# timmeinhardt/trackformer

Measured on AMD Instinct MI355X. Metric: frames/sec, TrackFormer-Deformable inference (ResNet-50, 1333x800, 300 object + 100 track queries, bs 1 per GPU); roofline = ms_deform_attn HBM GB/s, higher is better.
Workload: dtype f32 (dense layers as the fp16 split product on MFMA: two fp16 pieces per activation, three per weight scaled per output channel -- 22 + 1 significand bits per operand, the one dropped product < 2^-22 --, three terms, f32 accumulate)

## Files before the change

include/tf_fused.h:

```cpp
#ifndef TF_FUSED_H_
#define TF_FUSED_H_

#include <stdint.h>

#ifdef __cplusplus
extern "C" {
#endif

int tf_bias_act_f32(float *x, const float *bias, const float *residual, int64_t n, int C, int relu,
                    void *stream);

int tf_add_layernorm_f32(const float *x, const float *res, const float *gamma, const float *beta,
                         float *out, int64_t rows, int C, float eps, void *stream);

int tf_box_refine_f32(const float *delta, const float *ref, float *out, int64_t rows, int ref_dim, float eps, void *stream);

int tf_postprocess_pack_f32(const float *logits, const float *boxes, float *out, int64_t Q, int C, float img_h, float img_w,
                            int clip, void *stream);

int tf_groupnorm_nhwc_f32(const float *x, const float *gamma, const float *beta, float *out, double *workspace, int N,
                          int HW, int C, int G, float eps, int64_t x_image_stride, int64_t out_image_stride, void *stream);
int tf_groupnorm_stats_nhwc_f32(const float *x, double *workspace, int N, int HW, int C, int G, int64_t x_image_stride, void *stream);
int tf_groupnorm_relu_nhwc_f32(const float *x, const float *gamma, const float *beta, float *out, double *workspace, int N,
                               int HW, int C, int G, float eps, int64_t x_image_stride, int64_t out_image_stride, void *stream);

int tf_upsample_add_nhwc_f32(const float *low, const float *fpn, float *out, int N, int q_per_image, int h, int w, int H, int W, int C,
                             void *stream);

int tf_conv3x3_merge_packed_f32(const float *low, const float *fpn, const double *gn_workspace, const float *gamma, const float *beta,
                                int groups, float eps, const void *w_packed, const float *bias, float *y, int nimg, int q_per_image, int lh,
                                int lw, int H, int W, int cin, int cout, int relu, int terms, void *stream);

int tf_groupnorm_relu_conv3x3_c1_nhwc_f32(const float *x, const float *gamma, const float *beta, const float *weight, float bias,
                                          float *out, double *workspace, int N, int H, int W, int C, int G, float eps, void *stream);

int tf_mask_label_map_f32(const float *logits, const int *order, int16_t *label, int n_tracks, int h, int w, int pad_h, int pad_w, int img_h,
                          int img_w, int out_h, int out_w, float threshold, void *stream);


// ... 87 lines not shown
```

include/tf_msda.h:

```cpp
#ifndef TF_MSDA_H_
#define TF_MSDA_H_

#include <stdint.h>

#ifdef __cplusplus
extern "C" {
#endif

#define TF_MSDA_ABI_VERSION 8
#define TF_MSDA_MAX_LEVELS 16

typedef enum tf_msda_status {
    TF_MSDA_OK = 0,
    TF_MSDA_ERR_NULL_POINTER = -1,
    TF_MSDA_ERR_BAD_DIMS = -2,
    TF_MSDA_ERR_SHAPE_SUM = -3,
    TF_MSDA_ERR_LAUNCH = -4,
    TF_MSDA_ERR_NO_DEVICE = -5,
    TF_MSDA_ERR_WORKSPACE = -6
} tf_msda_status;

int tf_msda_abi_version(void);

const char *tf_msda_strerror(int status);
// ... 87 lines not shown
```

trackformer_amd/_cabi.py:

```python
import ctypes
import os

_PKG_DIR = os.path.dirname(os.path.abspath(__file__))
LIB_PATH = os.environ.get("TF_MSDA_LIB") or os.path.join(_PKG_DIR, "lib", "libtf_msda.so")

EXPORTED_SYMBOLS = (
    "tf_msda_abi_version",
    "tf_msda_strerror",
    "tf_msda_last_hip_error",
    "tf_msda_last_kernel",
    "tf_msda_set_tiled",
    "tf_msda_set_option",
    "tf_msda_debug_trace_buffer",
    "tf_msda_forward_fused_f32",
    "tf_msda_forward_f32",
    "tf_msda_forward_f64",
    "tf_msda_forward_f32_dshapes",
    "tf_msda_forward_f64_dshapes",
    "tf_msda_backward_f32",
    "tf_msda_backward_f64",
    "tf_msda_backward_f32_dshapes",
    "tf_msda_backward_f64_dshapes",
    "tf_msda_backward_det_workspace_bytes",
    "tf_msda_backward_det_f32",
    "tf_msda_backward_det_f64",
    "tf_msda_backward_det_f32_dshapes",
    "tf_msda_backward_det_f64_dshapes",
    "tf_msda_fused_prologue_f32",
    "tf_msda_fused_backward_epilogue_f32",
    "tf_msda_forward_host_f32",
    "tf_msda_forward_host_f64",
    "tf_msda_backward_host_f32",
    "tf_msda_backward_host_f64",
    "tf_bias_act_f32",
    "tf_add_layernorm_f32",
    "tf_groupnorm_nhwc_f32",
    "tf_groupnorm_relu_nhwc_f32",
    "tf_box_refine_f32",
    "tf_postprocess_pack_f32",
    "tf_upsample_add_nhwc_f32",
    "tf_mask_label_map_f32",
    "tf_conv3x3_merge_packed_f32",
    "tf_groupnorm_stats_nhwc_f32",
    "tf_groupnorm_relu_conv3x3_c1_nhwc_f32",
    "tf_bias_relu_maxpool_f32",
    "tf_stem_conv7x7_f32",
    "tf_linear_split_f32",
    "tf_linear_split_res_f32",
    "tf_conv3x3_split_f32",
    "tf_conv3x3_splitk_f32",
    "tf_conv1x1_strided_split_f32",
    "tf_conv1x1_splitk_f32",
# ... 8 lines not shown
    "tf_add_layernorm_train_f32",
    "tf_add_layernorm_bwd_workspace_bytes",
    "tf_add_layernorm_bwd_f32",
    "tf_set_criterion_fwd_f32",
    "tf_set_criterion_bwd_f32",
    "tf_match_cost_f32",
    "tf_linear_split_add_f32",
    "tf_ffn_fused_f32",
    "tf_linear_res_ln_f32",
    "tf_linear_groups_f32",
    "tf_conv_packed_f32",
    "tf_mha_core_f32",
    "tf_nms_host_f32",
)

ABI_VERSION = 8

_lib = None


class ProjGroup(ctypes.Structure):
    _fields_ = [("w_packed", ctypes.c_void_p), ("bias", ctypes.c_void_p), ("y", ctypes.c_void_p), ("N", ctypes.c_int),
                ("add_x2", ctypes.c_int)]


class MSDAError(RuntimeError):
    """Raised when libtf_msda.so reports a non-zero status."""


def lib():
    global _lib
# ... 61 lines not shown
    L.tf_postprocess_pack_f32.restype = ci
    L.tf_postprocess_pack_f32.argtypes = [vp, vp, vp, ctypes.c_int64, ci, ctypes.c_float, ctypes.c_float, ci, vp]
    L.tf_groupnorm_stats_nhwc_f32.restype = ci
    L.tf_groupnorm_stats_nhwc_f32.argtypes = [vp, vp, ci, ci, ci, ci, ctypes.c_int64, vp]
    L.tf_conv3x3_merge_packed_f32.restype = ci
    L.tf_conv3x3_merge_packed_f32.argtypes = [vp, vp, vp, vp, vp, ci, ctypes.c_float, vp, vp, vp, ci, ci, ci, ci, ci, ci, ci, ci, ci, ci, vp]
    L.tf_mask_label_map_f32.restype = ci
    L.tf_mask_label_map_f32.argtypes = [vp, vp, vp, ci, ci, ci, ci, ci, ci, ci, ci, ci, ctypes.c_float, vp]
    L.tf_upsample_add_nhwc_f32.restype = ci
    L.tf_upsample_add_nhwc_f32.argtypes = [vp, vp, vp, ci, ci, ci, ci, ci, ci, ci, vp]
    L.tf_groupnorm_relu_conv3x3_c1_nhwc_f32.restype = ci
    L.tf_groupnorm_relu_conv3x3_c1_nhwc_f32.argtypes = [vp, vp, vp, vp, ctypes.c_float, vp, vp, ci, ci, ci, ci, ci, ctypes.c_float, vp]
    for fn in (L.tf_groupnorm_nhwc_f32, L.tf_groupnorm_relu_nhwc_f32):
        fn.restype = ci
        fn.argtypes = [vp, vp, vp, vp, vp, ci, ci, ci, ci, ctypes.c_float, ctypes.c_int64, ctypes.c_int64, vp]
    L.tf_linear_split_f32.restype = ci
    L.tf_linear_split_f32.argtypes = [vp, vp, vp, vp, vp, vp, vp, ctypes.c_int64, ci, ci, ci, vp]
    L.tf_linear_split_res_f32.restype = ci
    L.tf_linear_split_res_f32.argtypes = [vp, vp, vp, vp, vp, vp, vp, vp, ctypes.c_int64, ci, ci, ci, vp]
    L.tf_conv3x3_splitk_f32.restype = ci
    L.tf_conv3x3_splitk_f32.argtypes = [vp, vp, vp, vp, vp, vp, vp, vp, ci, ci, ci, ci, ci, ci, ci, ci, vp]
    L.tf_conv3x3_split_f32.restype = ci
    L.tf_conv3x3_split_f32.argtypes = [vp, vp, vp, vp, vp, vp, vp] + [ci] * 7 + [vp]
    L.tf_conv1x1_splitk_f32.restype = ci
    L.tf_conv1x1_splitk_f32.argtypes = [vp, vp, vp, vp, vp, vp, vp, vp, ci, ci, ci, ci, ci, ci, ci, ci, vp]
    L.tf_conv1x1_strided_split_f32.restype = ci
    L.tf_conv1x1_strided_split_f32.argtypes = [vp, vp, vp, vp, vp, vp, vp] + [ci] * 7 + [vp]
    L.tf_linear_packed_bytes.restype = ctypes.c_int64
    L.tf_linear_packed_bytes.argtypes = [ci, ci, ci]
    L.tf_linear_pack_weight_f32.restype = ci
# ... 53 lines not shown
```

trackformer_amd/backbone.py:

```python
from collections import OrderedDict
from typing import Dict, List

import torch
import torch.nn.functional as F
from torch import nn

from . import fused
from .nested import NestedTensor, all_valid_mask, is_all_valid
from .position_encoding import build_position_encoding


import os as _os

CHANNELS_LAST = _os.environ.get("TF_BACKBONE_NCHW", "0") != "1"


_conv1x1_split = _os.environ.get("TF_CONV1X1_SPLIT", "1") != "0"


_conv3x3_split = _os.environ.get("TF_CONV3X3_SPLIT", "1") != "0"


def _parse_skip(text):
    out = set()
# ... 240 lines not shown
                return y
            y = y + b.reshape(1, -1, 1, 1)
        else:
            y = F.conv2d(x, cache.weight, b, conv.stride, conv.padding, conv.dilation, conv.groups)
        if residual is not None:
            y = y.add_(residual)
        return F.relu_(y) if relu else y
    if fold == 2 and not x.is_cuda:
        fold = 0
    x = bn(conv(x))
    if residual is not None:
        x = x + residual
    return F.relu(x) if relu else x


def _stem_pooled(x, conv1, bn1, maxpool, cache: _FoldCache):
    if not ((fused.stem_pool_fused_enabled() or fused.stem_conv_split_enabled()) and x.is_cuda and CHANNELS_LAST
            and isinstance(bn1, FrozenBatchNorm2d)
            and isinstance(maxpool, nn.MaxPool2d) and maxpool.kernel_size == 3 and maxpool.stride == 2
            and maxpool.padding == 1 and maxpool.dilation == 1 and not maxpool.ceil_mode):
        return None
    b = cache.get(conv1, bn1)
    w = cache.weight
    y = None
    if (conv1.kernel_size == (7, 7) and conv1.stride == (2, 2) and conv1.padding == (3, 3) and conv1.dilation == (1, 1)
            and conv1.groups == 1):
        fuse_pool = fused.stem_pool_fused_enabled()
        y = fused.stem_conv(x, w, None if fuse_pool else b, relu=not fuse_pool)
        if y is not None and not fuse_pool:
            return maxpool(y)
    if y is None:
        if not fused.stem_pool_fused_enabled():
            return None
        y = F.conv2d(x, w, None, conv1.stride, conv1.padding, conv1.dilation, conv1.groups)
    pooled = fused.bias_relu_maxpool(y, b)
    if pooled is None:
        if fused.bias_act_(y, b, None, True) is None:
            y = F.relu_(y + b.reshape(1, -1, 1, 1))
        pooled = maxpool(y)
    return pooled


class Bottleneck(nn.Module):
    expansion = 4

    def __init__(self, inplanes, planes, stride=1, downsample=None, dilation=1,
                 norm_layer=FrozenBatchNorm2d):
        super().__init__()
# ... 96 lines not shown

    def __init__(self, model: nn.Module, return_layers: Dict[str, str]):
        if not set(return_layers).issubset(name for name, _ in model.named_children()):
            raise ValueError("return_layers are not present in model")
        remaining = dict(return_layers)
        kept = OrderedDict()
        for name, module in model.named_children():
            kept[name] = module
            remaining.pop(name, None)
            if not remaining:
                break
        super().__init__(kept)
        self.return_layers = dict(return_layers)
        self._fold = _FoldCache()

    def forward(self, x):
        out = OrderedDict()
        fold = _fold_mode(self["conv1"], x) if (self.training and "conv1" in self) else int(_inference_mode(self))
        fused_stem = fold == 1 and all(k in self for k in ("conv1", "bn1", "relu"))
        pooled_stem = (fused_stem and "maxpool" in self
                       and not any(k in self.return_layers for k in ("conv1", "bn1", "relu", "maxpool")))
        skip = ()
        for name, module in self.items():
            if name in skip or (fused_stem and name in ("bn1", "relu")):
                continue
            if fused_stem and name == "conv1":
                pooled = _stem_pooled(x, self["conv1"], self["bn1"], self["maxpool"], self._fold) if pooled_stem else None
                if pooled is not None:
                    x, skip = pooled, ("maxpool",)
                    continue
                x = _conv_bn(x, self["conv1"], self["bn1"], self._fold, True, 1)
            else:
                x = module(x)
            if name in self.return_layers:
                out[self.return_layers[name]] = x
        return out


class BackboneBase(nn.Module):
    def __init__(self, backbone: nn.Module, train_backbone: bool, return_interm_layers: bool):
        super().__init__()
        for name, parameter in backbone.named_parameters():
            if not train_backbone or not any(k in name for k in ("layer2", "layer3", "layer4")):
                parameter.requires_grad_(False)
        if return_interm_layers:
            return_layers = {"layer1": "0", "layer2": "1", "layer3": "2", "layer4": "3"}
            self.strides = [4, 8, 16, 32]
            self.num_channels = [256, 512, 1024, 2048]
        else:
            return_layers = {"layer4": "0"}
            self.strides = [32]
            self.num_channels = [2048]
        self.body = IntermediateLayerGetter(backbone, return_layers=return_layers)

    def forward(self, tensor_list: NestedTensor):
        x = tensor_list.tensors
        if (_inference_mode(self) or (_train_fold and self.training)) and x.is_cuda and CHANNELS_LAST:
            x = x.contiguous(memory_format=torch.channels_last)
        xs = self.body(x)
        m = tensor_list.mask
        assert m is not None
        out: Dict[str, NestedTensor] = {}
        for name, feat in xs.items():
            if is_all_valid(m):
                mask = all_valid_mask((m.shape[0],) + tuple(feat.shape[-2:]), feat.device)
            else:
                mask = F.interpolate(m[None].float(), size=feat.shape[-2:]).to(torch.bool)[0]
            out[name] = NestedTensor(feat, mask)
        return out


class Backbone(BackboneBase):

    def __init__(self, name: str, train_backbone: bool, return_interm_layers: bool, dilation: bool):
# ... 31 lines not shown
```

trackformer_amd/build.py:

```python
import hashlib
import os
import shutil
import subprocess
import sys
from concurrent.futures import ThreadPoolExecutor

PKG_DIR = os.path.dirname(os.path.abspath(__file__))
REPO_DIR = os.path.dirname(PKG_DIR)
CSRC = os.path.join(PKG_DIR, "csrc")
LIB_DIR = os.path.join(PKG_DIR, "lib")
INCLUDE = os.path.join(REPO_DIR, "include")
GFX_ARCH = "gfx950"

_TARGETS = [
    ("libtf_msda.so", ["msda_hip.hip", "msda_pquad.hip", "fused_ops.hip", "linear_split.hip", "linear_stream.hip", "mha_core.hip", "ffn_fused.hip", "stem_conv.hip", "msda_host.cpp"], []),
]


def _hipcc():
    exe = shutil.which("hipcc") or "/opt/rocm/bin/hipcc"
    if not os.path.exists(exe):
        raise RuntimeError("hipcc not found (expected on PATH or at /opt/rocm/bin/hipcc)")
    return exe

# ... 45 lines not shown
        objs = [os.path.join(obj_dir, os.path.splitext(s)[0] + ".o") for s in srcs]
        with ThreadPoolExecutor(max_workers=len(srcs)) as pool:
            list(pool.map(lambda so: _run([_hipcc()] + flags + ["-c", so[0], "-o", so[1]], verbose),
                          zip(src_paths, objs)))
        _run([_hipcc(), "--offload-arch=" + GFX_ARCH, "-shared", "-fPIC", "-pthread"] + objs + ["-o", out], verbose)
        _stamp(out, key)
        built.append(out)
    built += _build_tools(force, verbose)
    return built


def _build_tools(force, verbose):
    out_dir = os.path.join(REPO_DIR, "tools", "bin")
    lib = os.path.join(LIB_DIR, "libtf_msda.so")
    built = []
    for name in ("msda_bench", "linear_bench", "ffn_bench", "proj_groups_bench"):
        src = os.path.join(REPO_DIR, "tools", name + ".cpp")
        if not os.path.exists(src):
            continue
        os.makedirs(out_dir, exist_ok=True)
        out = os.path.join(out_dir, name)
        flags = ["--offload-arch=" + GFX_ARCH, "-O2", "-std=c++17", "-I" + INCLUDE]
        headers = [os.path.join(INCLUDE, f) for f in os.listdir(INCLUDE) if f.endswith(".h")]
        key = _key([src] + headers, flags)
        if not force and not _stale(out, key) and os.path.getmtime(out) >= os.path.getmtime(lib):
            continue
        _run([_hipcc()] + flags + [src, "-L" + LIB_DIR, "-ltf_msda",
                                   "-Wl,-rpath,$ORIGIN/../../trackformer_amd/lib", "-o", out], verbose)
        _stamp(out, key)
        built.append(out)
    return built
# ... 6 lines not shown
```

trackformer_amd/csrc/fused_ops.hip:

```cpp
#include <hip/hip_runtime.h>

#include <stdint.h>
#include <stdlib.h>

#include <atomic>

#include "msda_common.h"
#include "tf_fused.h"
#include "tf_msda.h"

namespace {

typedef float f32x4_t __attribute__((ext_vector_type(4)));
typedef float f32x2_t __attribute__((ext_vector_type(2)));

template <bool RES, bool RELU>
__global__ void __launch_bounds__(256)
bias_act_kernel(float *__restrict__ x, const float *__restrict__ bias, const float *__restrict__ residual,
                        long long n4, int C4)
{
    const long long stride = (long long)gridDim.x * blockDim.x;
    const long long first = (long long)blockIdx.x * blockDim.x + threadIdx.x;
    const int step = (int)(stride % C4);
    int q0 = (int)(first % C4);
// ... 183 lines not shown
        f32x4_t y;
        y.x = (v.x - s_mean[g0]) * s_rstd[g0] * ga.x + be.x;
        y.y = (v.y - s_mean[g1]) * s_rstd[g1] * ga.y + be.y;
        y.z = (v.z - s_mean[g2]) * s_rstd[g2] * ga.z + be.z;
        y.w = (v.w - s_mean[g3]) * s_rstd[g3] * ga.w + be.w;
        if (RELU) {
            y.x = y.x < 0.f ? 0.f : y.x;
            y.y = y.y < 0.f ? 0.f : y.y;
            y.z = y.z < 0.f ? 0.f : y.z;
            y.w = y.w < 0.f ? 0.f : y.w;
        }
        tfm::stream_store(op + i, y);
    }
}

__global__ void __launch_bounds__(256)
upsample_add_nhwc_kernel(const float *__restrict__ low, const float *__restrict__ fpn, float *__restrict__ out, int q_per_image,
                         int h, int w, int H, int W, int C4, float sy, float sx, long long total)
{
    const long long stride = (long long)gridDim.x * blockDim.x;
    for (long long i = (long long)blockIdx.x * blockDim.x + threadIdx.x; i < total; i += stride) {
        const int c = (int)(i % C4);
        const long long p = i / C4;
        const int x = (int)(p % W);
        const long long q = p / W;
        const int y = (int)(q % H);
        const int n = (int)(q / H);
        const int ys = min((int)floorf((float)y * sy), h - 1), xs = min((int)floorf((float)x * sx), w - 1);
        const f32x4_t a = reinterpret_cast<const f32x4_t *>(low)[(((long long)n * h + ys) * w + xs) * C4 + c];
        const f32x4_t b = reinterpret_cast<const f32x4_t *>(fpn)[(((long long)(n / q_per_image) * H + y) * W + x) * C4 + c];
// ... 305 lines not shown
    const unsigned sblocks = (unsigned)((HW + kGnRowsPerBlock - 1) / kGnRowsPerBlock);
    hipLaunchKernelGGL(groupnorm_stats_kernel, dim3(sblocks, (unsigned)N), dim3(256), 0, s, x, workspace, HW, C, G, (long long)x_image_stride);
    return hipGetLastError() == hipSuccess ? TF_MSDA_OK : TF_MSDA_ERR_LAUNCH;
}

int tf_groupnorm_nhwc_f32(const float *x, const float *gamma, const float *beta, float *out, double *workspace, int N,
                          int HW, int C, int G, float eps, int64_t x_image_stride, int64_t out_image_stride, void *stream)
{
    return groupnorm_nhwc_impl(x, gamma, beta, out, workspace, N, HW, C, G, eps, x_image_stride, out_image_stride, false, stream);
}

int tf_groupnorm_relu_nhwc_f32(const float *x, const float *gamma, const float *beta, float *out, double *workspace, int N,
                               int HW, int C, int G, float eps, int64_t x_image_stride, int64_t out_image_stride, void *stream)
{
    return groupnorm_nhwc_impl(x, gamma, beta, out, workspace, N, HW, C, G, eps, x_image_stride, out_image_stride, true, stream);
}

int tf_bias_act_f32(float *x, const float *bias, const float *residual, int64_t n, int C, int relu,
                    void *stream)
{
    if (!x || !bias) return TF_MSDA_ERR_NULL_POINTER;
    if (n <= 0 || C <= 0 || (C & 3) || (n % C) != 0) return TF_MSDA_ERR_BAD_DIMS;
    if (!aligned16(x) || !aligned16(bias) || (residual && !aligned16(residual)))
        return TF_MSDA_ERR_BAD_DIMS;
    if (residual == x) return TF_MSDA_ERR_BAD_DIMS;
    const long long n4 = n / 4;
    long long blocks = (n4 + 255) / 256;
    if (blocks > 256 * 16) blocks = 256 * 16;
    hipStream_t s = static_cast<hipStream_t>(stream);
    if (residual && relu)
// ... 56 lines not shown
```

trackformer_amd/deformable_detr.py:

```python
import copy
import math

import torch
import torch.nn.functional as F
from torch import nn

from . import box_ops, fused
from .detr import DETR, PostProcess
from .nested import (NestedTensor, all_valid_mask, inverse_sigmoid, is_all_valid,
                     nested_tensor_from_tensor_list)


def _get_clones(module, N):
    return nn.ModuleList([copy.deepcopy(module) for _ in range(N)])


class DeformableDETR(DETR):
    track_query_filler_ok = True

    def __init__(self, backbone, transformer, num_classes, num_queries, num_feature_levels,
                 aux_loss=True, with_box_refine=False, two_stage=False, overflow_boxes=False,
                 multi_frame_attention=False, multi_frame_encoding=False,
                 merge_frame_features=False):
        super().__init__(backbone, transformer, num_classes, num_queries, aux_loss)
# ... 78 lines not shown
        query_embeds = None if self.two_stage else self.query_embed.weight
        hs, memory, init_reference, inter_references, enc_outputs_class, enc_outputs_coord_unact = \
            self.transformer.decode(enc, query_embeds, targets)
        return self._heads(hs, memory, init_reference, inter_references, enc_outputs_class, enc_outputs_coord_unact,
                           targets, features_all, src_shapes)

    def encode_frame(self, samples, prev_features=None):
        if not isinstance(samples, NestedTensor):
            samples = nested_tensor_from_tensor_list(samples)
        features_all, pos = self.backbone(samples)
        features = features_all[-3:]
        prev_features = features if prev_features is None else prev_features[-3:]

        frames = [prev_features, features] if self.multi_frame_attention else [features]
        src_list, mask_list, pos_list = [], [], []
        for frame, frame_feat in enumerate(frames):
            per_frame_pos = self.multi_frame_attention and self.multi_frame_encoding
            pos_list.extend([p[:, frame] for p in pos[-3:]] if per_frame_pos else pos[-3:])
            for lvl, feat in enumerate(frame_feat):
                src, mask = feat.decompose()
                assert mask is not None
                prev_src = prev_features[lvl].tensors if self.merge_frame_features else None
                src_list.append(self._project(lvl, src, prev_src))
                mask_list.append(mask)

            for lvl in range(len(frame_feat), self.num_feature_levels):
                if lvl == len(frame_feat):
                    src = self._project(lvl, frame_feat[-1].tensors,
                                        prev_features[-1].tensors if self.merge_frame_features
                                        else None)
                else:
                    src = self.input_proj[lvl](src_list[-1])
                m = frame_feat[0].mask
                if is_all_valid(m):
                    mask = all_valid_mask((m.shape[0],) + tuple(src.shape[-2:]), src.device)
                else:
                    mask = F.interpolate(m[None].float(), size=src.shape[-2:]).to(torch.bool)[0]
                pos_l = self.backbone[1](NestedTensor(src, mask)).to(src.dtype)
                src_list.append(src)
                mask_list.append(mask)
                pos_list.append(pos_l[:, frame] if per_frame_pos else pos_l)

        return {"features_all": features_all, "src_shapes": [tuple(s.shape[-2:]) for s in src_list],
                "enc": self.transformer.encode(src_list, mask_list, pos_list)}

    def _heads(self, hs, memory, init_reference, inter_references, enc_outputs_class, enc_outputs_coord_unact, targets,
               features_all, src_shapes):
        reuse_refinement = (self.with_box_refine and not self.two_stage and not self.training
                            and not torch.is_grad_enabled()
                            and inter_references.shape[0] == hs.shape[0])
        if reuse_refinement:
            outputs_coord = inter_references
            outputs_class = torch.stack([fused.head_linear(self.class_embed[lvl], hs[lvl])
                                         for lvl in range(hs.shape[0])])
        else:
            outputs_classes, outputs_coords = [], []
            for lvl in range(hs.shape[0]):
                reference = inverse_sigmoid(init_reference if lvl == 0
                                            else inter_references[lvl - 1])
# ... 44 lines not shown
```

trackformer_amd/deformable_transformer.py:

```python
import copy
import math

import torch
import torch.nn.functional as F
from torch import nn
from torch.nn.init import constant_, normal_, xavier_uniform_

from . import fused
from .msda import MSDeformAttn, attach_host_shapes
from .nested import inverse_sigmoid, is_all_valid


def _inference(module) -> bool:
    return (not module.training) and (not torch.is_grad_enabled())


def _ffn_hidden(linear, activation, x, inference):
    if inference and activation is F.relu and x.is_cuda and x.dtype == torch.float32:
        if fused.split_linear_enabled():
            y = fused.linear(x, linear.weight, linear.bias, relu=True)
            if y is not None:
                return y
        x2 = x.reshape(-1, x.shape[-1])
        y = torch._addmm_activation(linear.bias, x2, linear.weight.t(), use_gelu=False)
# ... 182 lines not shown
        key = tuple((id(p), p._version) for p in pos_embeds) + (id(self.level_embed), fused.source_key(self.level_embed))
        cache = self.__dict__.setdefault("_lvl_pos_cache", {})
        hit = cache.get(key)
        if hit is None:
            if (pos_embeds[0].is_cuda and torch.cuda.is_current_stream_capturing()) or len(cache) >= _KEEP_CACHE_ENTRIES:
                return compute()
            hit = (compute(), list(pos_embeds) + [self.level_embed])
            if pos_embeds[0].is_cuda:
                fused._publish_barrier(pos_embeds[0].device)
            cache[key] = hit
        return hit[0]

    def forward(self, srcs, masks, pos_embeds, query_embed=None, targets=None):
        return self.decode(self.encode(srcs, masks, pos_embeds), query_embed, targets)

    def encode(self, srcs, masks, pos_embeds):
        shapes = tuple((int(s.shape[2]), int(s.shape[3])) for s in srcs)
        device = srcs[0].device
        src_flatten = torch.cat([s.flatten(2).transpose(1, 2) for s in srcs], 1)
        lvl_pos_embed_flatten = self._level_position_embedding(pos_embeds)
        unpadded = all(is_all_valid(m) for m in masks)
        if unpadded:
            mask_flatten = None
            valid_ratios = _GEOMETRY.unit_valid_ratios(src_flatten.shape[0], len(shapes), device)
        else:
            mask_flatten = torch.cat([m.flatten(1) for m in masks], 1)
            valid_ratios = torch.stack([self.get_valid_ratio(m) for m in masks], 1)
        spatial_shapes = _GEOMETRY.spatial_shapes(shapes, device)

        if self.multi_frame_attention_separate_encoder:
            half_t = src_flatten.shape[1] // 2
            half_l = self.num_feature_levels // 2

            def run(sl_t, sl_l):
# ... 312 lines not shown
```

trackformer_amd/fused.py:

```python
import os
import threading

import torch
import torch.nn.functional as F

from . import _cabi


def _stream(device):
    return torch.cuda.current_stream(device).cuda_stream


def _param_ok(t, x):
    return (t.device == x.device and t.dtype == torch.float32 and t.is_contiguous()
            and t.data_ptr() % 16 == 0)


_weight_epoch = 0
_route_epoch = 0


def weight_epoch():
    return _weight_epoch

# ... 424 lines not shown
            return None
        w = weight.detach()
        w2 = torch.zeros((64, 176), dtype=torch.float32, device=w.device)
        w2[:, :168] = F.pad(w, (0, 1)).reshape(64, 168)
        nbytes = _cabi.lib().tf_linear_packed_bytes(176, 64, terms)
        with torch.cuda.device(w.device):
            packed = torch.empty(nbytes, dtype=torch.uint8, device=w.device)
            rc = _cabi.lib().tf_linear_pack_weight_f32(w2.data_ptr(), packed.data_ptr(), 176, 64, terms, _stream(w.device))
        _cabi.check(rc, "tf_linear_pack_weight_f32")
        _publish_barrier(w.device)
        hit = (key, packed)
        weight._tf_stem_packed = hit
    return hit[1]


def stem_conv(x, weight, bias=None, relu=False):
    if not (_stem_conv_split and _split_linear and x.is_cuda and x.dtype == torch.float32 and x.dim() == 4 and x.shape[1] == 3
            and tuple(weight.shape) == (64, 3, 7, 7) and weight.dtype == torch.float32 and weight.device == x.device
            and x.numel() > 0):
        return None
    if bias is not None and not (_param_ok(bias, x) and bias.numel() == 64):
        return None
    x = x if x.is_contiguous() else x.contiguous()
    n, _, h, w = x.shape
    ho, wo = (h - 1) // 2 + 1, (w - 1) // 2 + 1
    if n > 65535 or n * ho * wo * 256 >= 0xC0000000 or n * 3 * h * w >= 2 ** 31:
        return None
    packed = _stem_packed(weight)
    if packed is None:
        return None
    with torch.cuda.device(x.device):
        y = torch.empty((n, 64, ho, wo), dtype=torch.float32, device=x.device, memory_format=torch.channels_last)
        rc = _cabi.lib().tf_stem_conv7x7_f32(x.data_ptr(), packed.data_ptr(), 0 if bias is None else bias.data_ptr(), y.data_ptr(),
                                             n, h, w, 1 if relu else 0, _terms(), _stream(x.device))
# ... 401 lines not shown
    if hit is None or hit[0] != key or not same_sources(hit[3], srcs):
        if torch.cuda.is_current_stream_capturing():
            return None
        hit = conv._tf_c1_taps = (key, conv.weight.detach()[0].permute(1, 2, 0).reshape(9, c).contiguous(),
                                  0.0 if conv.bias is None else float(conv.bias.detach()), srcs)
    with torch.cuda.device(x.device):
        out = torch.empty((n, 1, H, W), dtype=torch.float32, device=x.device)
        ws = torch.empty(2 * n * gn.num_groups, dtype=torch.float64, device=x.device)
        rc = _cabi.lib().tf_groupnorm_relu_conv3x3_c1_nhwc_f32(x.data_ptr(), gn.weight.data_ptr(), gn.bias.data_ptr(), hit[1].data_ptr(), hit[2],
                                                               out.data_ptr(), ws.data_ptr(), n, H, W, c, gn.num_groups, float(gn.eps),
                                                               _stream(x.device))
    _cabi.check(rc, "tf_groupnorm_relu_conv3x3_c1_nhwc_f32")
    return out


def input_proj_1x1(x, conv, gn):
    if not (_input_proj_fused and _split_linear and x.is_cuda and x.dim() == 4 and x.dtype == torch.float32 and conv.groups == 1):
        return None
    if conv.kernel_size == (3, 3) and conv.stride == (2, 2) and conv.padding == (1, 1) and conv.dilation == (1, 1):
        if not x.is_contiguous(memory_format=torch.channels_last):
            x = x.contiguous(memory_format=torch.channels_last)
        cout, cin = conv.out_channels, conv.in_channels
        hit = getattr(conv, "_tf_wtaps", None)
        key = source_key(conv.weight)
        if hit is None or hit[0] != key or hit[2] is not conv.weight:
            prev_img = None if hit is None else hit[1]
            hit = (key, conv.weight.detach().permute(0, 2, 3, 1).reshape(cout, 9 * cin).contiguous(), conv.weight)
            inherit_route(hit[1], conv.weight, prev_img)
            conv._tf_wtaps = hit
        y = conv3x3(x, hit[1], conv.bias, False, 2)
        if y is None:
            return None
        n, _, ho, wo = y.shape
        z2 = groupnorm_nhwc(y.permute(0, 2, 3, 1).reshape(n * ho * wo, cout), n, gn)
        return None if z2 is None else z2.view(n, ho, wo, cout).permute(0, 3, 1, 2)
    if not (conv.kernel_size == (1, 1) and conv.stride == (1, 1) and conv.padding == (0, 0)):
        return None
    if not x.is_contiguous(memory_format=torch.channels_last):
        x = x.contiguous(memory_format=torch.channels_last)
    n, cin, h, w = x.shape
    cout = conv.out_channels
    hit = getattr(conv, "_tf_w2d", None)
    key = source_key(conv.weight)
    if hit is None or hit[0] != key or hit[2] is not conv.weight:
        prev_img = None if hit is None else hit[1]
        hit = (key, conv.weight.detach().reshape(cout, cin).contiguous(), conv.weight)
        inherit_route(hit[1], conv.weight, prev_img)
        if hit[1].is_cuda and hit[1].data_ptr() != conv.weight.data_ptr():
            _publish_barrier(hit[1].device)
        conv._tf_w2d = hit
    y2 = None
    if conv1x1_wants_split_k(n * h * w, cin, cout):
        y = conv3x3(x, hit[1], conv.bias, False, 1)
        y2 = None if y is None else y.permute(0, 2, 3, 1)
    if y2 is None:
        y2 = linear(x.permute(0, 2, 3, 1).reshape(n * h * w, cin), hit[1], conv.bias)
    if y2 is None:
        return None
    z2 = groupnorm_nhwc(y2.reshape(n * h * w, cout), n, gn)
    if z2 is None:
        return None
    return z2.view(n, h, w, cout).permute(0, 3, 1, 2)


_box_refine_fused = os.environ.get("TF_BOX_REFINE_FUSED", "1") != "0"


def set_box_refine_fused(on):
    global _box_refine_fused
    prev, _box_refine_fused = _box_refine_fused, bool(on)
    return _switched(prev, _box_refine_fused)


def box_refine(delta, reference_points):
    if not (_box_refine_fused and delta.is_cuda and delta.dtype == torch.float32 and reference_points.dtype == torch.float32
            and delta.shape[-1] == 4 and reference_points.shape[-1] in (2, 4)
            and delta.shape[:-1] == reference_points.shape[:-1] and delta.is_contiguous()
# ... 443 lines not shown
```

Measured before the change: 387.7.

## Batch input-projection GroupNorm across levels and write encoder-flattened output directly

Adds a multi-level GroupNorm path (stats, finish, apply kernels driven by a level table) so all input-projection levels are normalized in three launches instead of one per level. The result is written straight into the flattened [N, sum(HW), C] buffer that the encoder consumes, removing the per-level transpose and torch.cat copy. It also skips the up-front channels_last conversion of the input image when the split stem conv path applies, converting only on fallback. The cost is extra Python glue and ctypes pointer arrays on each call, and the fast path is only taken under a row-count threshold condition.

```diff
diff --git a/include/tf_fused.h b/include/tf_fused.h
--- a/include/tf_fused.h
+++ b/include/tf_fused.h
@@ -23,6 +23,11 @@
 int tf_groupnorm_stats_nhwc_f32(const float *x, double *workspace, int N, int HW, int C, int G, int64_t x_image_stride, void *stream);
 int tf_groupnorm_relu_nhwc_f32(const float *x, const float *gamma, const float *beta, float *out, double *workspace, int N,
                                int HW, int C, int G, float eps, int64_t x_image_stride, int64_t out_image_stride, void *stream);
+#define TF_GN_MAX_LEVELS 8
+int64_t tf_groupnorm_levels_workspace_bytes(const int *hw, int levels, int N, int G);
+int tf_groupnorm_levels_nhwc_f32(const float *const *x, const float *const *gamma, const float *const *beta, const int *hw, int levels,
+                                 float *out, void *workspace, int64_t workspace_bytes, int N, int C, int G, float eps,
+                                 int64_t out_image_stride, void *stream);
 
 int tf_upsample_add_nhwc_f32(const float *low, const float *fpn, float *out, int N, int q_per_image, int h, int w, int H, int W, int C,
                              void *stream);
diff --git a/include/tf_msda.h b/include/tf_msda.h
--- a/include/tf_msda.h
+++ b/include/tf_msda.h
@@ -7,7 +7,7 @@
 extern "C" {
 #endif
 
-#define TF_MSDA_ABI_VERSION 8
+#define TF_MSDA_ABI_VERSION 9
 #define TF_MSDA_MAX_LEVELS 16
 
 typedef enum tf_msda_status {
diff --git a/trackformer_amd/_cabi.py b/trackformer_amd/_cabi.py
--- a/trackformer_amd/_cabi.py
+++ b/trackformer_amd/_cabi.py
@@ -36,6 +36,8 @@
     "tf_add_layernorm_f32",
     "tf_groupnorm_nhwc_f32",
     "tf_groupnorm_relu_nhwc_f32",
+    "tf_groupnorm_levels_workspace_bytes",
+    "tf_groupnorm_levels_nhwc_f32",
     "tf_box_refine_f32",
     "tf_postprocess_pack_f32",
     "tf_upsample_add_nhwc_f32",
@@ -74,7 +76,7 @@
     "tf_nms_host_f32",
 )
 
-ABI_VERSION = 8
+ABI_VERSION = 9
 
 _lib = None
 
@@ -166,6 +168,10 @@
     for fn in (L.tf_groupnorm_nhwc_f32, L.tf_groupnorm_relu_nhwc_f32):
         fn.restype = ci
         fn.argtypes = [vp, vp, vp, vp, vp, ci, ci, ci, ci, ctypes.c_float, ctypes.c_int64, ctypes.c_int64, vp]
+    L.tf_groupnorm_levels_workspace_bytes.restype = ctypes.c_int64
+    L.tf_groupnorm_levels_workspace_bytes.argtypes = [vp, ci, ci, ci]
+    L.tf_groupnorm_levels_nhwc_f32.restype = ci
+    L.tf_groupnorm_levels_nhwc_f32.argtypes = [vp, vp, vp, vp, ci, vp, vp, ctypes.c_int64, ci, ci, ci, ctypes.c_float, ctypes.c_int64, vp]
     L.tf_linear_split_f32.restype = ci
     L.tf_linear_split_f32.argtypes = [vp, vp, vp, vp, vp, vp, vp, ctypes.c_int64, ci, ci, ci, vp]
     L.tf_linear_split_res_f32.restype = ci
diff --git a/trackformer_amd/backbone.py b/trackformer_amd/backbone.py
--- a/trackformer_amd/backbone.py
+++ b/trackformer_amd/backbone.py
@@ -278,7 +278,7 @@
     return F.relu(x) if relu else x
 
 
-def _stem_pooled(x, conv1, bn1, maxpool, cache: _FoldCache):
+def _stem_pooled(x, conv1, bn1, maxpool, cache: _FoldCache, to_channels_last=False):
     if not ((fused.stem_pool_fused_enabled() or fused.stem_conv_split_enabled()) and x.is_cuda and CHANNELS_LAST
             and isinstance(bn1, FrozenBatchNorm2d)
             and isinstance(maxpool, nn.MaxPool2d) and maxpool.kernel_size == 3 and maxpool.stride == 2
@@ -296,6 +296,8 @@
     if y is None:
         if not fused.stem_pool_fused_enabled():
             return None
+        if to_channels_last:
+            x = x.contiguous(memory_format=torch.channels_last)
         y = F.conv2d(x, w, None, conv1.stride, conv1.padding, conv1.dilation, conv1.groups)
     pooled = fused.bias_relu_maxpool(y, b)
     if pooled is None:
@@ -422,7 +424,7 @@
         self.return_layers = dict(return_layers)
         self._fold = _FoldCache()
 
-    def forward(self, x):
+    def forward(self, x, to_channels_last=False):
         out = OrderedDict()
         fold = _fold_mode(self["conv1"], x) if (self.training and "conv1" in self) else int(_inference_mode(self))
         fused_stem = fold == 1 and all(k in self for k in ("conv1", "bn1", "relu"))
@@ -433,12 +435,17 @@
             if name in skip or (fused_stem and name in ("bn1", "relu")):
                 continue
             if fused_stem and name == "conv1":
-                pooled = _stem_pooled(x, self["conv1"], self["bn1"], self["maxpool"], self._fold) if pooled_stem else None
+                pooled = (_stem_pooled(x, self["conv1"], self["bn1"], self["maxpool"], self._fold, to_channels_last)
+                          if pooled_stem else None)
                 if pooled is not None:
                     x, skip = pooled, ("maxpool",)
                     continue
+                if to_channels_last:
+                    x = x.contiguous(memory_format=torch.channels_last)
                 x = _conv_bn(x, self["conv1"], self["bn1"], self._fold, True, 1)
             else:
+                if to_channels_last and name == "conv1":
+                    x = x.contiguous(memory_format=torch.channels_last)
                 x = module(x)
             if name in self.return_layers:
                 out[self.return_layers[name]] = x
@@ -463,9 +470,12 @@
 
     def forward(self, tensor_list: NestedTensor):
         x = tensor_list.tensors
+        planar = False
         if (_inference_mode(self) or (_train_fold and self.training)) and x.is_cuda and CHANNELS_LAST:
-            x = x.contiguous(memory_format=torch.channels_last)
-        xs = self.body(x)
+            planar = "conv1" in self.body and x.is_contiguous() and fused.stem_conv_applies(x, self.body["conv1"].weight)
+            if not planar:
+                x = x.contiguous(memory_format=torch.channels_last)
+        xs = self.body(x, to_channels_last=planar) if planar else self.body(x)
         m = tensor_list.mask
         assert m is not None
         out: Dict[str, NestedTensor] = {}
diff --git a/trackformer_amd/build.py b/trackformer_amd/build.py
--- a/trackformer_amd/build.py
+++ b/trackformer_amd/build.py
@@ -83,7 +83,7 @@
     out_dir = os.path.join(REPO_DIR, "tools", "bin")
     lib = os.path.join(LIB_DIR, "libtf_msda.so")
     built = []
-    for name in ("msda_bench", "linear_bench", "ffn_bench", "proj_groups_bench"):
+    for name in ("msda_bench", "linear_bench", "ffn_bench", "proj_groups_bench", "gn_levels_bench"):
         src = os.path.join(REPO_DIR, "tools", name + ".cpp")
         if not os.path.exists(src):
             continue
diff --git a/trackformer_amd/csrc/fused_ops.hip b/trackformer_amd/csrc/fused_ops.hip
--- a/trackformer_amd/csrc/fused_ops.hip
+++ b/trackformer_amd/csrc/fused_ops.hip
@@ -221,6 +221,158 @@
     }
 }
 
+struct GnLevelTable {
+    const float *x[TF_GN_MAX_LEVELS];
+    const float *gamma[TF_GN_MAX_LEVELS];
+    const float *beta[TF_GN_MAX_LEVELS];
+    int hw[TF_GN_MAX_LEVELS];
+    int row0[TF_GN_MAX_LEVELS];
+    int chunk0[TF_GN_MAX_LEVELS + 1];
+    int ablock0[TF_GN_MAX_LEVELS + 1];
+    int levels;
+};
+
+constexpr int kGnApplyRows = 16;
+constexpr int kGnFinishBatch = 8;
+
+__device__ __forceinline__ int gn_level_of(const int *first, int levels, int b)
+{
+    int l = 0;
+    for (int i = 1; i < levels; ++i) l = b >= first[i] ? i : l;
+    return l;
+}
+
+__global__ void __launch_bounds__(256)
+gn_levels_stats_kernel(const GnLevelTable t, double *__restrict__ part, int C, int G)
+{
+    __shared__ double s_sum[1024], s_sq[1024];
+    const int C4 = C >> 2, cpg = C / G;
+    const int n = blockIdx.y;
+    const int l = gn_level_of(t.chunk0, t.levels, (int)blockIdx.x);
+    const int HW = t.hw[l];
+    const int r0 = ((int)blockIdx.x - t.chunk0[l]) * kGnRowsPerBlock, r1 = min(HW, r0 + kGnRowsPerBlock);
+    const int nslots = 256 / C4;
+    const int q = threadIdx.x % C4, rslot = threadIdx.x / C4;
+    if (rslot < nslots) {
+        const f32x4_t *xp = reinterpret_cast<const f32x4_t *>(t.x[l] + (long long)n * HW * C);
+        double s0 = 0.0, s1 = 0.0, s2 = 0.0, s3 = 0.0, q0 = 0.0, q1 = 0.0, q2 = 0.0, q3 = 0.0;
+        auto acc = [&](const f32x4_t &v) {
+            const double a = (double)v.x, b = (double)v.y, c = (double)v.z, d = (double)v.w;
+            s0 += a; s1 += b; s2 += c; s3 += d;
+            q0 = fma(a, a, q0); q1 = fma(b, b, q1); q2 = fma(c, c, q2); q3 = fma(d, d, q3);
+        };
+        int r = r0 + rslot;
+        for (; r + 3 * nslots < r1; r += 4 * nslots) {
+            const f32x4_t v0 = xp[(long long)r * C4 + q], v1 = xp[(long long)(r + nslots) * C4 + q];
+            const f32x4_t v2 = xp[(long long)(r + 2 * nslots) * C4 + q], v3 = xp[(long long)(r + 3 * nslots) * C4 + q];
+            acc(v0);
+            acc(v1);
+            acc(v2);
+            acc(v3);
+        }
+        for (; r < r1; r += nslots) acc(xp[(long long)r * C4 + q]);
+        double *ps = s_sum + rslot * C + 4 * q, *pq = s_sq + rslot * C + 4 * q;
+        ps[0] = s0; ps[1] = s1; ps[2] = s2; ps[3] = s3;
+        pq[0] = q0; pq[1] = q1; pq[2] = q2; pq[3] = q3;
+    }
+    __syncthreads();
+    for (int g = threadIdx.x; g < G; g += blockDim.x) {
+        double s = 0.0, sq = 0.0;
+        for (int c = g * cpg; c < (g + 1) * cpg; ++c)
+            for (int k = 0; k < nslots; ++k) {
+                s += s_sum[k * C + c];
+                sq += s_sq[k * C + c];
+            }
+        double *p = part + (((long long)n * t.chunk0[t.levels] + blockIdx.x) * G + g) * 2;
+        p[0] = s;
+        p[1] = sq;
+    }
+}
+
+__global__ void __launch_bounds__(256)
+gn_levels_finish_kernel(const GnLevelTable t, const double *__restrict__ part, f32x2_t *__restrict__ stat, int C, int G, float eps)
+{
+    __shared__ double s_part[2 * 256];
+    const int l = blockIdx.x, n = blockIdx.y;
+    const int c0 = t.chunk0[l], nc = t.chunk0[l + 1] - c0;
+    const int ranges = 256 / G;
+    const int g = threadIdx.x % G, rg = threadIdx.x / G;
+    const int per = (nc + ranges - 1) / ranges;
+    if (rg < ranges) {
+        const double *p = part + (((long long)n * t.chunk0[t.levels] + c0) * G + g) * 2;
+        const int b = min(nc, rg * per), e = min(nc, b + per);
+        double s = 0.0, sq = 0.0;
+        int c = b;
+        for (; c + kGnFinishBatch <= e; c += kGnFinishBatch) {
+            double vs[kGnFinishBatch], vq[kGnFinishBatch];
+#pragma unroll
+            for (int k = 0; k < kGnFinishBatch; ++k) {
+                vs[k] = p[(long long)(c + k) * G * 2];
+                vq[k] = p[(long long)(c + k) * G * 2 + 1];
+            }
+#pragma unroll
+            for (int k = 0; k < kGnFinishBatch; ++k) {
+                s += vs[k];
+                sq += vq[k];
+            }
+        }
+        for (; c < e; ++c) {
+            s += p[(long long)c * G * 2];
+            sq += p[(long long)c * G * 2 + 1];
+        }
+        s_part[(rg * G + g) * 2] = s;
+        s_part[(rg * G + g) * 2 + 1] = sq;
+    }
+    __syncthreads();
+    if (threadIdx.x < G) {
+        double s = 0.0, sq = 0.0;
+        for (int k = 0; k < ranges; ++k) {
+            s += s_part[(k * G + g) * 2];
+            sq += s_part[(k * G + g) * 2 + 1];
+        }
+        const double cnt = (double)t.hw[l] * (double)(C / G);
+        const double mean = s / cnt;
+        double var = sq / cnt - mean * mean;
+        if (var < 0.0) var = 0.0;
+        stat[((long long)n * t.levels + l) * G + g] = f32x2_t{(float)mean, (float)(1.0 / sqrt(var + (double)eps))};
+    }
+}
+
+__global__ void __launch_bounds__(256)
+gn_levels_apply_kernel(const GnLevelTable t, const f32x2_t *__restrict__ stat, float *__restrict__ out, int C, int G,
+                       long long out_image_stride)
+{
+    __shared__ float s_mean[256], s_rstd[256];
+    const int C4 = C >> 2, cpg = C / G;
+    const int n = blockIdx.y;
+    const int l = gn_level_of(t.ablock0, t.levels, (int)blockIdx.x);
+    for (int g = threadIdx.x; g < G; g += blockDim.x) {
+        const f32x2_t ms = stat[((long long)n * t.levels + l) * G + g];
+        s_mean[g] = ms.x;
+        s_rstd[g] = ms.y;
+    }
+    __syncthreads();
+    const int HW = t.hw[l];
+    const int r0 = ((int)blockIdx.x - t.ablock0[l]) * kGnApplyRows, rows = min(HW - r0, kGnApplyRows);
+    const f32x4_t *xp = reinterpret_cast<const f32x4_t *>(t.x[l] + ((long long)n * HW + r0) * C);
+    f32x4_t *op = reinterpret_cast<f32x4_t *>(out + (long long)n * out_image_stride + (long long)(t.row0[l] + r0) * C);
+    const f32x4_t *gp = reinterpret_cast<const f32x4_t *>(t.gamma[l]), *bp = reinterpret_cast<const f32x4_t *>(t.beta[l]);
+    const int n4 = rows * C4;
+#pragma unroll 4
+    for (int i = threadIdx.x; i < n4; i += 256) {
+        const int q = i % C4;
+        const int g0 = (q * 4) / cpg, g1 = (q * 4 + 1) / cpg, g2 = (q * 4 + 2) / cpg, g3 = (q * 4 + 3) / cpg;
+        const f32x4_t v = xp[i];
+        const f32x4_t ga = gp[q], be = bp[q];
+        f32x4_t y;
+        y.x = (v.x - s_mean[g0]) * s_rstd[g0] * ga.x + be.x;
+        y.y = (v.y - s_mean[g1]) * s_rstd[g1] * ga.y + be.y;
+        y.z = (v.z - s_mean[g2]) * s_rstd[g2] * ga.z + be.z;
+        y.w = (v.w - s_mean[g3]) * s_rstd[g3] * ga.w + be.w;
+        tfm::stream_store(op + i, y);
+    }
+}
+
 __global__ void __launch_bounds__(256)
 upsample_add_nhwc_kernel(const float *__restrict__ low, const float *__restrict__ fpn, float *__restrict__ out, int q_per_image,
                          int h, int w, int H, int W, int C4, float sy, float sx, long long total)
@@ -556,6 +708,72 @@
                                int HW, int C, int G, float eps, int64_t x_image_stride, int64_t out_image_stride, void *stream)
 {
     return groupnorm_nhwc_impl(x, gamma, beta, out, workspace, N, HW, C, G, eps, x_image_stride, out_image_stride, true, stream);
+}
+
+static bool gn_levels_plan(const int *hw, int levels, GnLevelTable &t)
+{
+    if (!hw || levels < 1 || levels > TF_GN_MAX_LEVELS) return false;
+    long long rows = 0, chunks = 0, ablocks = 0;
+    for (int l = 0; l < levels; ++l) {
+        if (hw[l] <= 0) return false;
+        t.hw[l] = hw[l];
+        t.row0[l] = (int)rows;
+        t.chunk0[l] = (int)chunks;
+        t.ablock0[l] = (int)ablocks;
+        rows += hw[l];
+        chunks += (hw[l] + kGnRowsPerBlock - 1) / kGnRowsPerBlock;
+        ablocks += (hw[l] + kGnApplyRows - 1) / kGnApplyRows;
+        if (rows >= (1LL << 31)) return false;
+    }
+    for (int l = levels; l <= TF_GN_MAX_LEVELS; ++l) {
+        t.chunk0[l] = (int)chunks;
+        t.ablock0[l] = (int)ablocks;
+        if (l < TF_GN_MAX_LEVELS) {
+            t.hw[l] = 0;
+            t.row0[l] = (int)rows;
+            t.x[l] = t.gamma[l] = t.beta[l] = nullptr;
+        }
+    }
+    t.levels = levels;
+    return true;
+}
+
+int64_t tf_groupnorm_levels_workspace_bytes(const int *hw, int levels, int N, int G)
+{
+    GnLevelTable t;
+    if (N <= 0 || N > 65535 || G <= 0 || G > 256 || !gn_levels_plan(hw, levels, t)) return -1;
+    return (int64_t)N * G * ((int64_t)t.chunk0[levels] * 2 * (int64_t)sizeof(double) + (int64_t)levels * 2 * (int64_t)sizeof(float));
+}
+
+int tf_groupnorm_levels_nhwc_f32(const float *const *x, const float *const *gamma, const float *const *beta, const int *hw, int levels,
+                                 float *out, void *workspace, int64_t workspace_bytes, int N, int C, int G, float eps,
+                                 int64_t out_image_stride, void *stream)
+{
+    if (!x || !gamma || !beta || !hw || !out || !workspace) return TF_MSDA_ERR_NULL_POINTER;
+    for (int l = 0; l < levels && l < TF_GN_MAX_LEVELS; ++l)
+        if (!x[l] || !gamma[l] || !beta[l]) return TF_MSDA_ERR_NULL_POINTER;
+    if (N <= 0 || C <= 0 || G <= 0 || G > 256 || C > 1024 || (C % G) != 0 || (C & 3) || N > 65535) return TF_MSDA_ERR_BAD_DIMS;
+    GnLevelTable t;
+    if (!gn_levels_plan(hw, levels, t)) return TF_MSDA_ERR_BAD_DIMS;
+    const long long rows = (long long)t.row0[levels - 1] + hw[levels - 1];
+    if (out_image_stride < rows * C || (out_image_stride & 3) || !aligned16(out) || !aligned16(workspace)) return TF_MSDA_ERR_BAD_DIMS;
+    for (int l = 0; l < levels; ++l) {
+        if (!aligned16(x[l]) || !aligned16(gamma[l]) || !aligned16(beta[l])) return TF_MSDA_ERR_BAD_DIMS;
+        t.x[l] = x[l];
+        t.gamma[l] = gamma[l];
+        t.beta[l] = beta[l];
+    }
+    if (workspace_bytes < tf_groupnorm_levels_workspace_bytes(hw, levels, N, G)) return TF_MSDA_ERR_WORKSPACE;
+    hipStream_t s = static_cast<hipStream_t>(stream);
+    double *part = static_cast<double *>(workspace);
+    f32x2_t *stat = reinterpret_cast<f32x2_t *>(part + (long long)N * t.chunk0[levels] * G * 2);
+    hipLaunchKernelGGL(gn_levels_stats_kernel, dim3((unsigned)t.chunk0[levels], (unsigned)N), dim3(256), 0, s, t, part, C, G);
+    if (hipGetLastError() != hipSuccess) return TF_MSDA_ERR_LAUNCH;
+    hipLaunchKernelGGL(gn_levels_finish_kernel, dim3((unsigned)levels, (unsigned)N), dim3(256), 0, s, t, (const double *)part, stat, C, G, eps);
+    if (hipGetLastError() != hipSuccess) return TF_MSDA_ERR_LAUNCH;
+    hipLaunchKernelGGL(gn_levels_apply_kernel, dim3((unsigned)t.ablock0[levels], (unsigned)N), dim3(256), 0, s, t, (const f32x2_t *)stat, out,
+                       C, G, (long long)out_image_stride);
+    return hipGetLastError() == hipSuccess ? TF_MSDA_OK : TF_MSDA_ERR_LAUNCH;
 }
 
 int tf_bias_act_f32(float *x, const float *bias, const float *residual, int64_t n, int C, int relu,
diff --git a/trackformer_amd/deformable_detr.py b/trackformer_amd/deformable_detr.py
--- a/trackformer_amd/deformable_detr.py
+++ b/trackformer_amd/deformable_detr.py
@@ -116,6 +116,9 @@
 
         frames = [prev_features, features] if self.multi_frame_attention else [features]
         src_list, mask_list, pos_list = [], [], []
+        src_flat, level_srcs = self._project_levels(frames), None
+        if src_flat is not None:
+            src_flat, level_srcs = src_flat
         for frame, frame_feat in enumerate(frames):
             per_frame_pos = self.multi_frame_attention and self.multi_frame_encoding
             pos_list.extend([p[:, frame] for p in pos[-3:]] if per_frame_pos else pos[-3:])
@@ -123,11 +126,13 @@
                 src, mask = feat.decompose()
                 assert mask is not None
                 prev_src = prev_features[lvl].tensors if self.merge_frame_features else None
-                src_list.append(self._project(lvl, src, prev_src))
+                src_list.append(level_srcs[len(src_list)] if level_srcs is not None else self._project(lvl, src, prev_src))
                 mask_list.append(mask)
 
             for lvl in range(len(frame_feat), self.num_feature_levels):
-                if lvl == len(frame_feat):
+                if level_srcs is not None:
+                    src = level_srcs[len(src_list)]
+                elif lvl == len(frame_feat):
                     src = self._project(lvl, frame_feat[-1].tensors,
                                         prev_features[-1].tensors if self.merge_frame_features
                                         else None)
@@ -144,7 +149,39 @@
                 pos_list.append(pos_l[:, frame] if per_frame_pos else pos_l)
 
         return {"features_all": features_all, "src_shapes": [tuple(s.shape[-2:]) for s in src_list],
-                "enc": self.transformer.encode(src_list, mask_list, pos_list)}
+                "enc": self.transformer.encode(src_list, mask_list, pos_list, src_flat=src_flat)}
+
+    def _project_levels(self, frames):
+        feats = frames[0]
+        if not (fused.input_proj_levels_enabled() and not self.training and not torch.is_grad_enabled()
+                and not self.merge_frame_features and not self.multi_frame_attention and feats[0].tensors.is_cuda
+                and len(feats) <= self.num_feature_levels <= len(feats) + 1
+                and len(frames) * self.num_feature_levels <= fused.GN_MAX_LEVELS):
+            return None
+        n = feats[0].tensors.shape[0]
+        hw = [tuple(f.tensors.shape[-2:]) for f in feats]
+        if self.num_feature_levels > len(feats):
+            hw.append(((hw[-1][0] - 1) // 2 + 1, (hw[-1][1] - 1) // 2 + 1))
+        if len(frames) * sum(h * w for h, w in hw) < fused.input_proj_levels_min_rows():
+            return None
+        raws, shapes, norms = [], [], []
+        for frame_feat in frames:
+            for lvl in range(self.num_feature_levels):
+                x = frame_feat[min(lvl, len(frame_feat) - 1)].tensors
+                raw = fused.input_proj_raw(x, self.input_proj[lvl][0])
+                if raw is None:
+                    return None
+                raws.append(raw[0])
+                shapes.append(raw[1])
+                norms.append(self.input_proj[lvl][1])
+        flat = fused.groupnorm_levels(raws, n, norms)
+        if flat is None:
+            return None
+        views, row = [], 0
+        for h, w in shapes:
+            views.append(flat[:, row:row + h * w].view(n, h, w, flat.shape[2]).permute(0, 3, 1, 2))
+            row += h * w
+        return flat, views
 
     def _heads(self, hs, memory, init_reference, inter_references, enc_outputs_class, enc_outputs_coord_unact, targets,
                features_all, src_shapes):
diff --git a/trackformer_amd/deformable_transformer.py b/trackformer_amd/deformable_transformer.py
--- a/trackformer_amd/deformable_transformer.py
+++ b/trackformer_amd/deformable_transformer.py
@@ -220,10 +220,10 @@
     def forward(self, srcs, masks, pos_embeds, query_embed=None, targets=None):
         return self.decode(self.encode(srcs, masks, pos_embeds), query_embed, targets)
 
-    def encode(self, srcs, masks, pos_embeds):
+    def encode(self, srcs, masks, pos_embeds, src_flat=None):
         shapes = tuple((int(s.shape[2]), int(s.shape[3])) for s in srcs)
         device = srcs[0].device
-        src_flatten = torch.cat([s.flatten(2).transpose(1, 2) for s in srcs], 1)
+        src_flatten = src_flat if src_flat is not None else torch.cat([s.flatten(2).transpose(1, 2) for s in srcs], 1)
         lvl_pos_embed_flatten = self._level_position_embedding(pos_embeds)
         unpadded = all(is_all_valid(m) for m in masks)
         if unpadded:
diff --git a/trackformer_amd/fused.py b/trackformer_amd/fused.py
--- a/trackformer_amd/fused.py
+++ b/trackformer_amd/fused.py
@@ -1,3 +1,4 @@
+import ctypes
 import os
 import threading
 
@@ -462,10 +463,14 @@
     return hit[1]
 
 
+def stem_conv_applies(x, weight):
+    return bool(_stem_conv_split and _split_linear and x.is_cuda and x.dtype == torch.float32 and x.dim() == 4 and x.shape[1] == 3
+                and tuple(weight.shape) == (64, 3, 7, 7) and weight.dtype == torch.float32 and weight.device == x.device
+                and x.numel() > 0)
+
+
 def stem_conv(x, weight, bias=None, relu=False):
-    if not (_stem_conv_split and _split_linear and x.is_cuda and x.dtype == torch.float32 and x.dim() == 4 and x.shape[1] == 3
-            and tuple(weight.shape) == (64, 3, 7, 7) and weight.dtype == torch.float32 and weight.device == x.device
-            and x.numel() > 0):
+    if not stem_conv_applies(x, weight):
         return None
     if bias is not None and not (_param_ok(bias, x) and bias.numel() == 64):
         return None
@@ -897,7 +902,7 @@
     return out
 
 
-def input_proj_1x1(x, conv, gn):
+def input_proj_raw(x, conv):
     if not (_input_proj_fused and _split_linear and x.is_cuda and x.dim() == 4 and x.dtype == torch.float32 and conv.groups == 1):
         return None
     if conv.kernel_size == (3, 3) and conv.stride == (2, 2) and conv.padding == (1, 1) and conv.dilation == (1, 1):
@@ -915,8 +920,7 @@
         if y is None:
             return None
         n, _, ho, wo = y.shape
-        z2 = groupnorm_nhwc(y.permute(0, 2, 3, 1).reshape(n * ho * wo, cout), n, gn)
-        return None if z2 is None else z2.view(n, ho, wo, cout).permute(0, 3, 1, 2)
+        return y.permute(0, 2, 3, 1).reshape(n * ho * wo, cout), (ho, wo)
     if not (conv.kernel_size == (1, 1) and conv.stride == (1, 1) and conv.padding == (0, 0)):
         return None
     if not x.is_contiguous(memory_format=torch.channels_last):
@@ -940,10 +944,78 @@
         y2 = linear(x.permute(0, 2, 3, 1).reshape(n * h * w, cin), hit[1], conv.bias)
     if y2 is None:
         return None
-    z2 = groupnorm_nhwc(y2.reshape(n * h * w, cout), n, gn)
+    return y2.reshape(n * h * w, cout), (h, w)
+
+
+def input_proj_1x1(x, conv, gn):
+    raw = input_proj_raw(x, conv)
+    if raw is None:
+        return None
+    y2, (h, w) = raw
+    n = x.shape[0]
+    z2 = groupnorm_nhwc(y2, n, gn)
     if z2 is None:
         return None
-    return z2.view(n, h, w, cout).permute(0, 3, 1, 2)
+    return z2.view(n, h, w, conv.out_channels).permute(0, 3, 1, 2)
+
+
+_input_proj_levels = os.environ.get("TF_INPUT_PROJ_LEVELS", "1") != "0"
+_input_proj_levels_min_rows = int(os.environ.get("TF_INPUT_PROJ_LEVELS_MIN_ROWS", "4096"))
+
+
+def input_proj_levels_enabled():
+    return _input_proj_levels
+
+
+def input_proj_levels_min_rows():
+    return _input_proj_levels_min_rows
+
+
+def set_input_proj_levels_min_rows(n):
+    global _input_proj_levels_min_rows
+    prev, _input_proj_levels_min_rows = _input_proj_levels_min_rows, int(n)
+    return _switched(prev, _input_proj_levels_min_rows)
+
+
+def set_input_proj_levels(on):
+    global _input_proj_levels
+    prev, _input_proj_levels = _input_proj_levels, bool(on)
+    return _switched(prev, _input_proj_levels)
+
+
+GN_MAX_LEVELS = 8
+
+
+def groupnorm_levels(xs, n_img, gns):
+    if not (0 < len(xs) <= GN_MAX_LEVELS and len(gns) == len(xs)):
+        return None
+    x0, g0 = xs[0], gns[0]
+    c = g0.num_channels
+    if c % 4 or c > 1024 or g0.num_groups > 256 or not 0 < n_img <= 65535:
+        return None
+    for x2, gn in zip(xs, gns):
+        if not (x2.is_cuda and x2.dtype == torch.float32 and x2.dim() == 2 and x2.is_contiguous() and x2.device == x0.device
+                and x2.shape[1] == c and x2.shape[0] > 0 and x2.shape[0] % n_img == 0 and not (x2.data_ptr() & 15)
+                and gn.num_channels == c and gn.num_groups == g0.num_groups and gn.eps == g0.eps
+                and gn.weight is not None and gn.bias is not None and _param_ok(gn.weight, x0) and _param_ok(gn.bias, x0)):
+            return None
+    levels = len(xs)
+    hw = (ctypes.c_int * levels)(*[x2.shape[0] // n_img for x2 in xs])
+    if sum(hw) >= 2 ** 31:
+        return None
+    ptrs = lambda ts: (ctypes.c_void_p * levels)(*[t.data_ptr() for t in ts])
+    L = _cabi.lib()
+    nbytes = L.tf_groupnorm_levels_workspace_bytes(hw, levels, n_img, g0.num_groups)
+    if nbytes < 0:
+        return None
+    with torch.cuda.device(x0.device):
+        out = torch.empty((n_img, sum(hw), c), dtype=torch.float32, device=x0.device)
+        ws = torch.empty(nbytes // 8, dtype=torch.float64, device=x0.device)
+        rc = L.tf_groupnorm_levels_nhwc_f32(ptrs(xs), ptrs([gn.weight for gn in gns]), ptrs([gn.bias for gn in gns]), hw, levels,
+                                            out.data_ptr(), ws.data_ptr(), nbytes, n_img, c, g0.num_groups, float(g0.eps),
+                                            sum(hw) * c, _stream(x0.device))
+    _cabi.check(rc, "tf_groupnorm_levels_nhwc_f32")
+    return out
 
 
 _box_refine_fused = os.environ.get("TF_BOX_REFINE_FUSED", "1") != "0"
```

New measurement: 391.2, median of 6. About the same (+0.9%).
